# marcin119a/vae-los-angeles

Measured on AMD Instinct MI355X. Metric: training samples/sec, MultiModalVAE batch 65536, higher is better.
Workload: dtype bf16

## Files before the change

### include/mmvae_hip.h

```cpp
#ifndef MMVAE_HIP_H
#define MMVAE_HIP_H
#include <stdint.h>

#ifdef __cplusplus
extern "C" {
#endif

#define MMVAE_OK 0
#define MMVAE_ERR_ARG (-1)
#define MMVAE_ERR_DTYPE (-2)

enum { MMVAE_F32 = 0, MMVAE_BF16 = 1 };
enum { MMVAE_PREC_F32 = 0, MMVAE_PREC_BF16 = 1 };
enum { MMVAE_PRO_NONE = 0, MMVAE_PRO_BN_RELU_DROP = 1, MMVAE_PRO_BN_BWD_APPLY = 2 };
enum { MMVAE_EPI_STORE = 0, MMVAE_EPI_RELU_MASK = 1, MMVAE_EPI_BN_BWD = 2, MMVAE_EPI_LOSS_MSE = 3, MMVAE_EPI_LOSS_BCE_LOGIT = 4 };
enum { MMVAE_ACT_NONE = 0, MMVAE_ACT_RELU = 1, MMVAE_ACT_SIGMOID = 2 };

#define MMVAE_TILE 128

int mmvae_abi_version(void);
int mmvae_set_tuning(int32_t key, int32_t value);

typedef struct {
    const float* src; void* dst;
// ... 82 lines not shown

typedef struct {
    int32_t B, L, n_mod;
    const float* g_mu; const float* g_lv;
    const float* dz; const float* dz2; const float* dz3; int64_t lddz;
    const float* eps; const float* logvar;
    float* d_heads; int64_t ld_heads;
    float* d_table; const int64_t* site; int32_t S;
    void* d_heads_lp; int64_t ld_heads_lp;
    int32_t table_copies;
} mmvae_fuse_bwd_args;
#define MMVAE_TABLE_COPIES 8
int mmvae_fuse_reparam_bwd(const mmvae_fuse_bwd_args* args, void* stream);

typedef struct {
    int32_t B, A, D, S, L;
    const float* recon_a; const void* a; int64_t ld_ra, ld_a;
    const float* recon_b; const void* b; int64_t ld_rb, ld_b;
    const float* logits; int64_t ld_logits; const int64_t* site; const float* class_weights;
    const float* mu; const float* logvar;
    float beta, gamma;
    double* sums;
    void* g_a; int32_t g_a_dtype; int64_t ld_ga;
    void* g_b; int32_t g_b_dtype; int64_t ld_gb; int32_t grad_b_wrt_logit;
    float* g_c; int64_t ld_gc;
    float* g_mu; float* g_lv;
    const float* beta_gamma_dev;
    int32_t a_dtype, b_dtype;
} mmvae_loss_args;
int mmvae_vae_loss(const mmvae_loss_args* args, void* stream);
// ... 33 lines not shown
```

### vae-los-angeles_amd/csrc/common.h

```cpp
#pragma once
#include <hip/hip_runtime.h>
#include <stdint.h>
#include "mmvae_hip.h"

namespace mm {

typedef __bf16 bf16;
typedef __attribute__((ext_vector_type(8))) __bf16 bf16x8;
typedef __attribute__((ext_vector_type(4))) __bf16 bf16x4;
typedef __attribute__((ext_vector_type(4))) float f32x4;
typedef __attribute__((ext_vector_type(2))) float f32x2;
typedef __attribute__((ext_vector_type(4))) short s16x4;

constexpr int WAVE = 64;
constexpr int TILE = 128;
constexpr int NTHREADS = 256;
constexpr int ROW_BYTES = 128;

template <typename CT> struct Mma;

template <> struct Mma<bf16> {
    static constexpr int EPC = 8;
    static constexpr int KSTEP = 32;
    typedef bf16x8 frag;
// ... 123 lines not shown
#define STAMP_BUFFER(name)
#define STAMP_ENTRY()
#endif


struct Tuning {
    int nt_wide_min_m = 256 * 128;
    int nt2_on = 1;
    long split_bytes = 1L << 32;
    long block_bytes = 1L << 31;
    int tn_wide_on = 1;
    int bnbwd_stream = 1;
    int relu_stream = 1;
    int ntp_on = 1;
    int ntp_min_m = 16384;
};
inline Tuning g_tuning;

constexpr int NOT_TAKEN = 1 << 30;

template <auto Kernel, typename... Args>
inline int launch_lds(dim3 grid, dim3 block, int lds, hipStream_t st, const Args&... args) {
    static bool attr_done = false;
    if (!attr_done) {
        hipError_t e = hipFuncSetAttribute((const void*)Kernel, hipFuncAttributeMaxDynamicSharedMemorySize, lds);
        if (e != hipSuccess) return (int)e;
        attr_done = true;
    }
    hipLaunchKernelGGL(Kernel, grid, block, lds, st, args...);
    return (int)hipGetLastError();
// ... 49 lines not shown
```

### vae-los-angeles_amd/csrc/elementwise.hip

```cpp
#include <vector>
#include "common.h"
#include "mmvae_hip.h"

namespace mm {

__global__ __launch_bounds__(256) void prep_weights_kernel(const mmvae_prep_item* __restrict__ items) {
    const mmvae_prep_item it = items[blockIdx.y];
    __shared__ float tile[32][33];
    const int tx = threadIdx.x & 31, ty = threadIdx.x >> 5;
    const int tiles_c = (it.dst_cols + 31) / 32, tiles_r = (it.dst_rows + 31) / 32;
    auto put = [&](int r, int c, float v) {
        if (it.dst_dtype == MMVAE_BF16) ((bf16*)it.dst)[(long)r * it.dst_ld + c] = (bf16)v;
        else ((float*)it.dst)[(long)r * it.dst_ld + c] = v;
    };
    for (int t = blockIdx.x; t < tiles_r * tiles_c; t += gridDim.x) {
        const int tr = t / tiles_c, tc = t - tr * tiles_c;
        if (it.transpose) {
#pragma unroll
            for (int k = 0; k < 4; ++k) {
                const int sr = tc * 32 + ty + 8 * k, sc = tr * 32 + tx;
                tile[ty + 8 * k][tx] = (sr < it.src_rows && sc < it.src_cols) ? it.src[(long)sr * it.src_ld + sc] : 0.f;
            }
            __syncthreads();
#pragma unroll
// ... 189 lines not shown
    const float inv_n = 1.f / (float)a.n_mod;
    for (long i = (long)blockIdx.x * blockDim.x + threadIdx.x; i < total; i += (long)gridDim.x * blockDim.x) {
        const int b = (int)(i / a.ldz), l = (int)(i % a.ldz);
        ZT* zp = (ZT*)a.z + i;
        if (l >= a.L) { *zp = from_f32<ZT>(0.f); continue; }
        float mu = 0.f, lv = 0.f;
        if (a.heads_a) { mu += a.heads_a[(long)b * a.ld_heads + l]; lv += a.heads_a[(long)b * a.ld_heads + a.L + l]; }
        if (a.heads_b) { mu += a.heads_b[(long)b * a.ld_heads + l]; lv += a.heads_b[(long)b * a.ld_heads + a.L + l]; }
        if (a.table) {
            const long s = a.site[b];
            const bool ok = s >= 0 && s < a.S;
            const long sc = ok ? s : 0;
            const float bad = ok ? 0.f : __builtin_nanf("");
            mu += a.table[sc * 2 * a.L + l] + bad; lv += a.table[sc * 2 * a.L + a.L + l] + bad;
        }
        if (a.n_mod > 1) { mu *= inv_n; lv *= inv_n; }
        a.mu[(long)b * a.L + l] = mu; a.logvar[(long)b * a.L + l] = lv;
        *zp = from_f32<ZT>(mu + a.eps[(long)b * a.L + l] * expf(0.5f * lv));
    }
}

__global__ __launch_bounds__(256) void fuse_bwd_kernel(mmvae_fuse_bwd_args a, int rows_per_block, int use_lds) {
    extern __shared__ float sT[];
    const int L2 = 2 * a.L;
    if (use_lds) { for (int i = threadIdx.x; i < a.S * L2; i += blockDim.x) sT[i] = 0.f; __syncthreads(); }
    const int b0 = blockIdx.x * rows_per_block, b1 = min(a.B, b0 + rows_per_block);
    float* dtab = a.d_table ? a.d_table + (long)(blockIdx.x % (a.table_copies > 0 ? a.table_copies : 1)) * a.S * L2 : nullptr;
    const float inv_n = 1.f / (float)a.n_mod;
    constexpr int U = 4;
    const long iend = (long)b1 * a.L;
    for (long i0 = (long)b0 * a.L + threadIdx.x; i0 < iend; i0 += (long)U * blockDim.x) {
        float dz[U], gm[U], gl[U], ep[U], lv[U];
        int bb[U], ll[U];
// ... 772 lines not shown
```

### vae-los-angeles_amd/csrc/gemm_nt.hip

```cpp
#include "common.h"
#include "mmvae_hip.h"
#include "gemm_src.h"
#include "gemm_nt_epi.h"
#include "gemm_nt2.h"

namespace mm {

STAMP_BUFFER(nt)

__device__ __forceinline__ int swz(int row, int chunk) { return row * ROW_BYTES + ((chunk ^ (row & 7)) << 4); }

template <int WN> struct NtLds {
    static constexpr int BUF = (TILE + 64 * WN) * ROW_BYTES;
    static constexpr int STAGE = 2 * BUF;
    static constexpr int ECOL = STAGE + 4096 + 4 * 64 * WN * 4;
    static constexpr int TOTAL = ECOL + 8 * 64 * WN * 4;
};

template <typename CT, typename Src, typename Epi, int WN>
__global__ __launch_bounds__(128 * WN, 2)
void gemm_nt_kernel(Src src, const CT* __restrict__ W, long ldw, int M, int N, int K, int gx, int gy, Epi epi)
{
    constexpr int EPC = Mma<CT>::EPC;
    constexpr int BK = ROW_BYTES / (int)sizeof(CT);
// ... 245 lines not shown
                                    return launch_nt2<EpiLoss<MODE, VT, TT>, 2>(src.p, src.lda, a->w, a->ldw, a->M, a->N, a->K, e, st); }
#define MM_LOSS_VT(MODE, TT) { if (vt == 4) MM_LOSS_EPI(MODE, 4, TT) if (vt == 2) MM_LOSS_EPI(MODE, 2, TT) MM_LOSS_EPI(MODE, 1, TT) }
            if (h16) { if (mse) MM_LOSS_VT(0, bf16) MM_LOSS_VT(1, bf16) }
            if (mse) MM_LOSS_VT(0, float)
            MM_LOSS_VT(1, float)
#undef MM_LOSS_VT
#undef MM_LOSS_EPI
        }
        return MMVAE_ERR_ARG;
    }
    }
    return MMVAE_ERR_ARG;
}

BnFin bn_fin_of(const mmvae_gemm_nt_args* a) {
    BnFin f;
    if (!a->pro_finalize) return f;
    const mmvae_bn_finalize_args* b = (const mmvae_bn_finalize_args*)a->pro_finalize;
    f.sum = b->sum; f.sumsq = b->sumsq; f.gamma = b->gamma; f.beta = b->beta; f.eps = b->eps; f.momentum = b->momentum;
    f.running_mean = b->running_mean; f.running_var = b->running_var; f.nbt = (long long*)b->num_batches_tracked;
    f.mean = b->mean; f.rstd = b->rstd; f.scale = b->scale; f.shift = b->shift; f.M = b->M;
    return f;
}
static bool bn_fin_ok(const mmvae_gemm_nt_args* a) {
    if (!a->pro_finalize) return true;
    const mmvae_bn_finalize_args* b = (const mmvae_bn_finalize_args*)a->pro_finalize;
    return a->prologue == MMVAE_PRO_BN_RELU_DROP && b->N == a->K && b->M >= 2 && b->sum && b->sumsq && b->gamma && b->beta && b->mean && b->rstd && b->scale && b->shift;
}

template <typename CT>
static int dispatch_src(const mmvae_gemm_nt_args* a, hipStream_t st) {
    constexpr int EPC = Mma<CT>::EPC;
    if (a->prologue == MMVAE_PRO_BN_RELU_DROP) {
        if ((a->a_dtype == MMVAE_BF16) != (sizeof(CT) == 2)) return MMVAE_ERR_DTYPE;
        if (a->K > 512 || a->lda % EPC || ((uintptr_t)a->a & 15) || (!a->pro_finalize && (!a->pro_scale || !a->pro_shift))) return MMVAE_ERR_ARG;
        if (a->pro_mask && (a->ld_pro_mask % 4 || ((uintptr_t)a->pro_mask & 3))) return MMVAE_ERR_ARG;
        SrcBnReluDrop<CT> s{(const CT*)a->a, a->lda, a->M, a->K, a->pro_scale, a->pro_shift, a->pro_mask, a->ld_pro_mask, a->pro_inv_keep, bn_fin_of(a)};
// ... 15 lines not shown
extern "C" int mmvae_set_tuning(int32_t key, int32_t value) {
    mm::Tuning& t = mm::g_tuning;
    switch (key) {
    case 0: t.nt_wide_min_m = value; return 0;
    case 2: t.nt2_on = value; return 0;
    case 3:
        if (value != 0 && (value < 17 || value > 32)) return MMVAE_ERR_ARG;
        t.split_bytes = value ? 1L << value : mm::Tuning{}.split_bytes;
        t.block_bytes = t.split_bytes / 2;
        return 0;
    case 4: t.tn_wide_on = value; return 0;
    case 6: t.bnbwd_stream = value; return 0;
    case 7: t.relu_stream = value; return 0;
    case 8: t.ntp_on = value; return 0;
    case 9: t.ntp_min_m = value; return 0;
    }
    return MMVAE_ERR_ARG;
}

extern "C" int mmvae_gemm_nt(const mmvae_gemm_nt_args* a, void* stream) {
    if (!a || !a->a || !a->w || (!a->c && !(a->epilogue == MMVAE_EPI_BN_BWD && a->bn_phase == 0))) return MMVAE_ERR_ARG;
    if (a->M <= 0 || a->N <= 0 || a->K <= 0) return MMVAE_ERR_ARG;
    if (a->ldw % 64 || ((uintptr_t)a->w & 15)) return MMVAE_ERR_ARG;
    const long lim = 1L << 32;
    if (((long)a->N + 256) * a->ldw * 4 >= lim) return MMVAE_ERR_ARG;
    const long a_row = (long)a->lda * (a->a_dtype == MMVAE_BF16 ? 2 : 4);
    long row_bytes = a_row > (long)a->ld_pro_mask ? a_row : (long)a->ld_pro_mask;
    if (!mm::bn_fin_ok(a)) return MMVAE_ERR_ARG;
    if (mm::needs_row_blocks(a->M, row_bytes)) {
        if (a->pro_finalize || a->pro_out) return MMVAE_ERR_ARG;
// ... 23 lines not shown
```

### vae-los-angeles_amd/csrc/gemm_src.h

```cpp
#pragma once
#include "common.h"

namespace mm {

template <typename AT, int EPC> struct RawVec;
template <> struct RawVec<bf16, 8> {
    bf16x8 v;
    __device__ __forceinline__ float get(int i) const { return (float)v[i]; }
};
template <int EPC> struct RawVec<float, EPC> {
    float v[EPC];
    __device__ __forceinline__ float get(int i) const { return v[i]; }
};

template <int EPC, int VEC>
__device__ __forceinline__ void load_chunk_f32(RawVec<float, EPC>& r, const float* p, unsigned row_off, int k, int K) {
#pragma unroll
    for (int j = 0; j < EPC; j += VEC) VLoad<float, VEC>::ld(p + (row_off + (unsigned)min(k + j, K - VEC)), &r.v[j]);
}

template <typename CT, typename AT, int VEC>
struct SrcPlain {
    static constexpr int EPC = Mma<CT>::EPC;
    static constexpr bool NEEDS_AUX = false;
// ... 66 lines not shown
        if (var < 0.0) var = 0.0;
        const float rs = (float)(1.0 / sqrt(var + (double)eps));
        sc = gamma[i] * rs; sh = beta[i] - (float)mean_ * sc;
        if (first_wg) {
            mean[i] = (float)mean_; rstd[i] = rs; scale[i] = sc; shift[i] = sh;
            if (running_mean) {
                running_mean[i] = (1.f - momentum) * running_mean[i] + momentum * (float)mean_;
                const double unbiased = var * ((double)M / (double)(M - 1));
                running_var[i] = (1.f - momentum) * running_var[i] + momentum * (float)unbiased;
            }
            if (i == 0 && nbt) *nbt += 1;
        }
    }
};

template <typename CT>
struct SrcBnReluDrop {
    static constexpr int EPC = Mma<CT>::EPC;
    static constexpr bool NEEDS_AUX = true;
    static constexpr bool PAD_TAIL = false;
    const CT* y; long ldy; int M, K;
    const float* scale; const float* shift;
    const uint8_t* mask; long ldm; float inv_keep;
    BnFin fin = BnFin{};
    struct Raw { RawVec<CT, EPC> y; uint32_t m[EPC / 4]; };
    __device__ __forceinline__ void init(float* aux, int tid, int) const {
        if (fin.sum) {
            const bool first_wg = (blockIdx.x | blockIdx.y | blockIdx.z) == 0;
            for (int i = tid; i < K; i += NTHREADS) { float sc, sh; fin.column(i, first_wg, sc, sh); aux[i] = sc * inv_keep; aux[512 + i] = sh * inv_keep; }
            return;
// ... 84 lines not shown
```

### vae-los-angeles_amd/mmvae/_lib.py

```python
import ctypes as C
import os

_HERE = os.path.dirname(os.path.abspath(__file__))
LIB_PATH = os.environ.get("MMVAE_LIB_PATH") or os.path.join(_HERE, "libmmvae_hip.so")
ABI_VERSION = 20

F32, BF16 = 0, 1
PREC_F32, PREC_BF16 = 0, 1
PRO_NONE, PRO_BN_RELU_DROP, PRO_BN_BWD_APPLY = 0, 1, 2
TABLE_COPIES = 8
EPI_STORE, EPI_RELU_MASK, EPI_BN_BWD, EPI_LOSS_MSE, EPI_LOSS_BCE_LOGIT = 0, 1, 2, 3, 4
ACT_NONE, ACT_RELU, ACT_SIGMOID = 0, 1, 2
TILE = 128
TN_GROUP_MAX = 8
CTR_COPIES = 16384

i32, i64, f32, vp = C.c_int32, C.c_int64, C.c_float, C.c_void_p


class PrepItem(C.Structure):
    _fields_ = [("src", vp), ("dst", vp), ("src_rows", i32), ("src_cols", i32), ("src_ld", i64),
                ("dst_rows", i32), ("dst_cols", i32), ("dst_ld", i64), ("transpose", i32), ("dst_dtype", i32)]


# ... 38 lines not shown


class BnBwdFinalizeArgs(C.Structure):
    _fields_ = [("M", i32), ("N", i32), ("sum_d", vp), ("sum_dx", vp),
                ("gamma", vp), ("rstd", vp), ("dgamma", vp), ("dbeta", vp), ("coef", vp), ("eval_mode", i32)]


class FuseFwdArgs(C.Structure):
    _fields_ = [("B", i32), ("L", i32), ("n_mod", i32),
                ("heads_a", vp), ("heads_b", vp), ("ld_heads", i64),
                ("table", vp), ("site", vp), ("S", i32),
                ("eps", vp), ("mu", vp), ("logvar", vp),
                ("z", vp), ("z_dtype", i32), ("ldz", i64)]


class FuseBwdArgs(C.Structure):
    _fields_ = [("B", i32), ("L", i32), ("n_mod", i32),
                ("g_mu", vp), ("g_lv", vp), ("dz", vp), ("dz2", vp), ("dz3", vp), ("lddz", i64),
                ("eps", vp), ("logvar", vp),
                ("d_heads", vp), ("ld_heads", i64),
                ("d_table", vp), ("site", vp), ("S", i32), ("d_heads_lp", vp), ("ld_heads_lp", i64), ("table_copies", i32)]


class LossArgs(C.Structure):
    _fields_ = [("B", i32), ("A", i32), ("D", i32), ("S", i32), ("L", i32),
                ("recon_a", vp), ("a", vp), ("ld_ra", i64), ("ld_a", i64),
                ("recon_b", vp), ("b", vp), ("ld_rb", i64), ("ld_b", i64),
                ("logits", vp), ("ld_logits", i64), ("site", vp), ("class_weights", vp),
                ("mu", vp), ("logvar", vp),
                ("beta", f32), ("gamma", f32),
# ... 15 lines not shown
_SIGNATURES = {
    "mmvae_set_tuning": [i32, i32],
    "mmvae_prep_weights": [vp, i32, vp],
    "mmvae_gemm_nt": [C.POINTER(GemmNtArgs), vp],
    "mmvae_gemm_tn": [C.POINTER(GemmTnArgs), vp],
    "mmvae_gemm_tn_group": [vp, i32, vp],
    "mmvae_bn_finalize": [C.POINTER(BnFinalizeArgs), vp],
    "mmvae_bn_eval_coeffs": [i32, vp, vp, vp, vp, f32, vp, vp, vp, vp, vp],
    "mmvae_bn_bwd_finalize": [C.POINTER(BnBwdFinalizeArgs), vp],
    "mmvae_bn_bwd_apply": [i32, i32, i32, vp, i64, vp, i64, vp, vp, vp, vp],
    "mmvae_bn_bwd_finalize_apply": [i32, i32, i32, vp, i64, vp, i64, vp, vp, vp, vp, vp, vp, vp, i32, vp],
    "mmvae_embed_table_fwd": [i32, i32, i32, vp, vp, vp, vp, vp, vp, vp],
    "mmvae_embed_table_bwd": [i32, i32, i32, vp, vp, vp, vp, i32, vp, vp, vp, vp, vp, vp],
    "mmvae_fuse_reparam_fwd": [C.POINTER(FuseFwdArgs), vp],
    "mmvae_fuse_reparam_bwd": [C.POINTER(FuseBwdArgs), vp],
    "mmvae_vae_loss": [C.POINTER(LossArgs), vp],
    "mmvae_loss_finalize": [vp, f32, f32, vp, vp, vp],
    "mmvae_gather_rows": [vp, i32, vp, i32, i64, vp],
    "mmvae_rows_to_bf16": [vp, i32, i64, vp, i64, i32, i32, vp],
    "mmvae_sigmoid_bwd": [i32, i32, vp, i64, vp, i64, vp, i32, i64, vp],
    "mmvae_scale_if_needed": [vp, i32, i64, vp, vp],
    "mmvae_scale_many": [C.POINTER(ScaleItem), i32, vp, vp],
    "mmvae_noise": [vp, i64, f32, vp, i64, C.c_uint64, C.c_uint64, vp, i32, vp],
    "mmvae_counter_add": [vp, C.c_uint64, vp],
    "mmvae_adamw_step": [vp, i32, f32, f32, f32, f32, f32, f32, f32, i32, vp, i32, vp, vp],
}
EXPORTED = ["mmvae_abi_version"] + sorted(_SIGNATURES)

_lib = None

# ... 37 lines not shown
```

### vae-los-angeles_amd/mmvae/engine.py

```python
import os
from dataclasses import dataclass
from typing import NamedTuple, Optional

import torch

from . import ops
from . import _lib as L_
from .ops import (PREC_BF16, PREC_F32, ACT_NONE, ACT_RELU, ACT_SIGMOID, EPI_RELU_MASK, EPI_BN_BWD, DROP_P,
                  ceil_to, act_dtype, Prologue, BnBwdEpilogue, BnBwdFinalize, BnBwdApply)

_PRECISIONS = {"bf16": PREC_BF16, "fp32": PREC_F32, "f32": PREC_F32}
_default_precision = _PRECISIONS[os.environ.get("MMVAE_PRECISION", "bf16").lower()]
_TINY_DW_MAX = 16384


def set_default_precision(name):
    global _default_precision
    _default_precision = _PRECISIONS[name.lower()]


def default_precision():
    return _default_precision


# ... 184 lines not shown
        self.pl = [ops.PreparedLinear([l.weight], [l.bias], prec, device) for l in self.linears]
        self.pl_heads = ops.PreparedLinear([self.fc_mu.weight, self.fc_logvar.weight],
                                           [self.fc_mu.bias, self.fc_logvar.bias], prec, device)
        return self.pl + [self.pl_heads]

    def params(self):
        out = []
        for l, bn in zip(self.linears, self.bns):
            out += [l.weight, l.bias, bn.weight, bn.bias]
        out += [self.fc_mu.weight, self.fc_logvar.weight, self.fc_mu.bias, self.fc_logvar.bias]
        return out

    def widths(self):
        return [l.out_features for l in self.linears]

    def forward(self, prec, x, train, masks, stats_bufs=None, want_bwd=False):
        B, dev = x.shape[0], x.device
        adt = act_dtype(prec)
        layers = []
        h, pro = x, None
        fin = None

        def consume(N, K, out, bias, w, tag, stats=None, pro_out=None):
            nonlocal fin
            if fin is not None:
                try:
                    ops.gemm_nt(prec, h, w, N, K, out, bias=bias, prologue=pro, stats=stats, tag=tag, pro_out=pro_out, pro_finalize=fin)
                    fin = None
                    return pro_out
                except L_.MMVAEArgError:
                    pass
            if fin is not None:
                ops.bn_finalize_launch(fin)
                fin = None
            try:
                ops.gemm_nt(prec, h, w, N, K, out, bias=bias, prologue=pro, stats=stats, tag=tag, pro_out=pro_out)
                return pro_out
            except L_.MMVAEArgError:
                if pro_out is None:
                    raise
                ops.gemm_nt(prec, h, w, N, K, out, bias=bias, prologue=pro, stats=stats, tag=tag)
                return None

        for lin, bn, pl in zip(self.linears, self.bns, self.pl):
            N, K = pl.N, pl.K
            y = torch.empty(B, ceil_to(N, 8), dtype=adt, device=dev)
            st = BNState(N, dev)
            h_act = None
            if want_bwd and pro is not None and ops.can_keep_pro_out(prec, B, N, K, h, y) and pro.mask is not None \
                    and pro.mask.stride(0) % 8 == 0 and pro.mask.data_ptr() % 8 == 0:
                h_act = torch.empty(B, K, dtype=torch.bfloat16, device=dev)
            if train:
                stats = stats_bufs[len(layers)] if stats_bufs is not None else torch.zeros(2, N, dtype=torch.float64, device=dev)
                h_act = consume(N, K, y, pl.bias, pl.w, f"{self.name}.L{len(layers)}.fwd", stats=stats, pro_out=h_act)
                fin = ops.bn_finalize_args(B, N, stats, bn.weight, bn.bias, bn.running_mean, bn.running_var,
                                           bn.num_batches_tracked, st.mean, st.rstd, st.scale, st.shift, bn.eps,
                                           bn.momentum if bn.momentum is not None else 0.1)
                new_pro = Prologue(st.scale, st.shift, masks[len(layers)], 1.0 / (1.0 - DROP_P))
            else:
                ops.gemm_nt(prec, h, pl.w, N, K, y, bias=pl.bias, prologue=pro, tag=f"{self.name}.L{len(layers)}.fwd")
                ops.bn_eval_coeffs(bn.weight, bn.bias, bn.running_mean, bn.running_var, st.scale, st.shift, bn.eps, st.mean, st.rstd)
                new_pro = Prologue(st.scale, st.shift, None, 1.0)
            layers.append(LayerSave(h, pro, y, st, new_pro) if h_act is None else LayerSave(h_act, None, y, st, new_pro))
            h, pro = y, new_pro
        heads = torch.empty(B, 2 * self.latent, dtype=torch.float32, device=dev)
        consume(2 * self.latent, self.pl_heads.K, heads, self.pl_heads.bias, self.pl_heads.w, f"{self.name}.heads.fwd")
        return heads, layers

    def backward(self, prec, layers, d_heads, grads, tn=ops.gemm_tn, stats_bufs=None, train=True, d_heads_lp=None):
        B, dev = d_heads.shape[0], d_heads.device
        adt = act_dtype(prec)
        L2 = 2 * self.latent
        Kl = self.pl_heads.K
        gw = grads[self.fc_mu.weight]
        gb = grads[self.fc_mu.bias]
        tn(prec, d_heads, layers[-1].y, _span(gw, L2 * Kl).view(L2, Kl), _span(gb, L2), L2, Kl, q_prologue=layers[-1].y_prologue, tag=f"{self.name}.heads.dW")
        src, src_wt, src_n, src_k = (d_heads_lp if d_heads_lp is not None else d_heads), self.pl_heads.wt, Kl, L2
        for i in reversed(range(len(self.linears))):
            lin, bn, pl = self.linears[i], self.bns[i], self.pl[i]
            sv = layers[i]
            y = sv.y
            st = sv.bn
# ... 203 lines not shown

    def _forward(self, prec, xa, xb, site, train, want_bwd):
        ref = xa if xa is not None else (xb if xb is not None else site)
        dev, B = ref.device, ref.shape[0]
        self._prep.ensure(prec, dev, self.param_list(), self._prepare)
        state = StepState(prec, B, train)
        heads_a = heads_b = table = None
        Ld = self.latent
        widths_a = self.enc_a.widths() if (train and xa is not None) else []
        widths_b = self.enc_b.widths() if (train and xb is not None) else []
        n_a = len(widths_a)
        masks, eps = self.noise.draw(B, widths_a + widths_b, Ld, dev)
        zeros = self.zero_pack(dev, xa is not None, xb is not None, site is not None, fwd=True, bwd=want_bwd) if train else None
        if want_bwd:
            state.zeros = zeros
        if xa is not None:
            xa = _check_input(xa, "a", self.enc_a.in_dim, prec)
            heads_a, state.enc_a = self.enc_a.forward(prec, xa, train, masks[:n_a] if train else None,
                                                      zeros.fwd_stats[:n_a] if train else None, want_bwd=want_bwd)
        if xb is not None:
            xb = _check_input(xb.reshape(xb.shape[0], -1), "b", self.enc_b.in_dim, prec)
            heads_b, state.enc_b = self.enc_b.forward(prec, xb, train, masks[n_a:] if train else None,
                                                      zeros.fwd_stats[n_a:] if train else None, want_bwd=want_bwd)
        if site is not None:
            if site.dtype != torch.int64:
                site = site.long()
            site = site.contiguous()
            table = self.enc_c.table()
            state.site = site
        mu = torch.empty(B, Ld, dtype=torch.float32, device=dev)
        logvar = torch.empty(B, Ld, dtype=torch.float32, device=dev)
        z = torch.empty(B, ceil_to(Ld, 8), dtype=act_dtype(prec), device=dev)
        ops.fuse_reparam_fwd(B, Ld, heads_a, heads_b, table, site, eps, mu, logvar, z)
        state.eps, state.logvar = eps, logvar.detach()
        state.n_mod = (heads_a is not None) + (heads_b is not None) + (table is not None)
        outs, state.dec = [None] * len(self.decoders), [None] * len(self.decoders)
        order = sorted(range(len(self.decoders)), key=lambda i: -sum(l.weight.numel() for l in self.decoders[i].linears))
        stem = self.dec_stem
        firsts = [None] * len(self.decoders)
        if stem is not None:
            H0 = torch.empty(B, stem.N, dtype=act_dtype(prec), device=dev)
            ops.gemm_nt(prec, z, stem.w, stem.N, stem.K, H0, bias=stem.bias, act=ACT_RELU, tag="Decoders.L0.fwd")
            off = 0
            for i, d in enumerate(self.decoders):
                firsts[i] = H0[:, off:off + d.linears[0].out_features]
                off += d.linears[0].out_features
        fused = None
        want = self.fused_recon
        if want is not None and any(t is not None and self.decoders[i].can_fuse_loss(prec) for i, t in enumerate(want)):
            fused = state.fused = FusedRecon(*(zeros.loss_ws if want_bwd else ops.loss_workspace(dev)), {}, {})
        for i in order:
            dec = self.decoders[i]
            tgt = want[i] if (fused is not None and want[i] is not None and dec.can_fuse_loss(prec)) else None
            if tgt is not None:
                k = 1 if dec.final_sigmoid else 0
                g, acts = dec.forward(prec, z, fused_loss=(tgt, fused.sums[k:k + 1]), first=firsts[i])
                fused.g[i], fused.targets[i] = g, tgt
# ... 76 lines not shown
```

### vae-los-angeles_amd/mmvae/ops.py

```python
import ctypes as C
from collections import namedtuple

import torch

from . import _lib as L
from ._lib import (F32, BF16, PREC_F32, PREC_BF16, PRO_NONE, PRO_BN_RELU_DROP, PRO_BN_BWD_APPLY, EPI_STORE, EPI_RELU_MASK,
                   EPI_BN_BWD, EPI_LOSS_MSE, EPI_LOSS_BCE_LOGIT, ACT_NONE, ACT_RELU, ACT_SIGMOID, TILE)

DROP_P = 0.1
BN_EPS, BN_MOMENTUM = 1e-5, 0.1


class KernelProbe:

    def __init__(self, only=None):
        self.records = {}
        self.only = only

    def wants(self, tag):
        return tag is not None and (self.only is None or tag in self.only)

    def begin(self):
        ev = torch.cuda.Event(enable_timing=True)
        ev.record(torch.cuda.current_stream())
# ... 364 lines not shown
    L.check(L.load().mmvae_embed_table_bwd(S, E, w_mu.shape[0], emb.data_ptr(), w_mu.data_ptr(), w_lv.data_ptr(),
                                           d_table.data_ptr(), copies, d_emb.data_ptr(), d_w_mu.data_ptr(), d_b_mu.data_ptr(),
                                           d_w_lv.data_ptr(), d_b_lv.data_ptr(), _stream()), "mmvae_embed_table_bwd")


def fuse_reparam_fwd(B, Ld, heads_a, heads_b, table, site, eps, mu, logvar, z):
    n_mod = (heads_a is not None) + (heads_b is not None) + (table is not None)
    hd = heads_a if heads_a is not None else heads_b
    a = L.FuseFwdArgs(B, Ld, n_mod, _p(heads_a), _p(heads_b), _ld(hd) if hd is not None else 0,
                      _p(table), _p(site), table.shape[0] if table is not None else 0,
                      eps.data_ptr(), mu.data_ptr(), logvar.data_ptr(), z.data_ptr(), _dt(z), _ld(z))
    with stream_span("fuse_reparam_fwd", B * (8 * Ld * (n_mod - (table is not None)) + 8 * (table is not None) + 12 * Ld + z.element_size() * _ld(z))):
        L.check(L.load().mmvae_fuse_reparam_fwd(C.byref(a), _stream()), "mmvae_fuse_reparam_fwd")


def fuse_reparam_bwd(B, Ld, n_mod, g_mu, g_lv, dzs, eps, logvar, d_heads, d_table, site, d_heads_lp=None):
    dzs = list(dzs) + [None] * (3 - len(dzs))
    copies = d_table.shape[0] if (d_table is not None and d_table.dim() == 3) else 1
    a = L.FuseBwdArgs(B, Ld, n_mod, _p(g_mu), _p(g_lv), dzs[0].data_ptr(), _p(dzs[1]), _p(dzs[2]), _ld(dzs[0]), eps.data_ptr(), logvar.data_ptr(),
                      d_heads.data_ptr(), _ld(d_heads), _p(d_table), _p(site), d_table.shape[-2] if d_table is not None else 0,
                      _p(d_heads_lp), _ld(d_heads_lp) if d_heads_lp is not None else 0, copies)
    n_dz = sum(1 for d in dzs if d is not None)
    with stream_span("fuse_reparam_bwd", B * Ld * 4 * (n_dz + (g_mu is not None) + (g_lv is not None) + 2 + 2)):
        L.check(L.load().mmvae_fuse_reparam_bwd(C.byref(a), _stream()), "mmvae_fuse_reparam_bwd")


def loss_workspace(device):
    buf = torch.zeros(5 * 8 + 5 * 4 + 4, dtype=torch.uint8, device=device)
    return buf[:40].view(torch.float64), buf[40:60].view(torch.float32)

# ... 122 lines not shown
```

Measured before the change: 51.86 million.

## Fuse encoder heads, reparameterization and decoder stem into one latent kernel

Adds a single HIP kernel that applies the last encoder BN/ReLU/dropout prologue, computes both encoder head GEMMs, adds the site-embedding table, performs the reparameterization, writes mu/logvar/z, and runs the decoder stem GEMM with ReLU into H0. In the bf16 path this replaces separate head GEMMs, the fuse_reparam kernel and the stem GEMM, removing several launches and the round-trips of heads and z through global memory. If the kernel's argument checks fail, it falls back to the old sequence. The trade-offs are heavy LDS use and a persistent grid capped at 256 blocks, which may limit occupancy.

Measured after the change: 53.02 million (median of 6 runs). 2.3% higher.

```diff
diff --git a/include/mmvae_hip.h b/include/mmvae_hip.h
--- a/include/mmvae_hip.h
+++ b/include/mmvae_hip.h
@@ -120,6 +120,25 @@
 int mmvae_fuse_reparam_bwd(const mmvae_fuse_bwd_args* args, void* stream);
 
 typedef struct {
+    const void* y; int64_t ldy; int32_t K;
+    const float* scale; const float* shift;
+    const uint8_t* mask; int64_t ld_mask; float inv_keep;
+    const void* finalize;
+    const void* w; int64_t ldw; const float* bias;
+} mmvae_latent_enc;
+typedef struct {
+    int32_t prec, B, L, n_mod;
+    mmvae_latent_enc enc_a, enc_b;
+    const float* table; const int64_t* site; int32_t S;
+    const float* eps;
+    float* mu; float* logvar;
+    void* z; int64_t ldz;
+    const void* w_stem; int64_t ldw_stem; const float* bias_stem; int32_t N_stem;
+    void* h0; int64_t ldh0;
+} mmvae_latent_fwd_args;
+int mmvae_latent_fwd(const mmvae_latent_fwd_args* args, void* stream);
+
+typedef struct {
     int32_t B, A, D, S, L;
     const float* recon_a; const void* a; int64_t ld_ra, ld_a;
     const float* recon_b; const void* b; int64_t ld_rb, ld_b;
diff --git a/vae-los-angeles_amd/csrc/common.h b/vae-los-angeles_amd/csrc/common.h
--- a/vae-los-angeles_amd/csrc/common.h
+++ b/vae-los-angeles_amd/csrc/common.h
@@ -161,6 +161,7 @@
     int relu_stream = 1;
     int ntp_on = 1;
     int ntp_min_m = 16384;
+    int latent_on = 1;
 };
 inline Tuning g_tuning;
 
diff --git a/vae-los-angeles_amd/csrc/elementwise.hip b/vae-los-angeles_amd/csrc/elementwise.hip
--- a/vae-los-angeles_amd/csrc/elementwise.hip
+++ b/vae-los-angeles_amd/csrc/elementwise.hip
@@ -1,6 +1,7 @@
 #include <vector>
 #include "common.h"
 #include "mmvae_hip.h"
+#include "fuse_math.h"
 
 namespace mm {
 
@@ -227,9 +228,9 @@
             const float bad = ok ? 0.f : __builtin_nanf("");
             mu += a.table[sc * 2 * a.L + l] + bad; lv += a.table[sc * 2 * a.L + a.L + l] + bad;
         }
-        if (a.n_mod > 1) { mu *= inv_n; lv *= inv_n; }
+        const float zf = fuse_reparam_elem(mu, lv, a.n_mod, inv_n, a.eps[(long)b * a.L + l]);
         a.mu[(long)b * a.L + l] = mu; a.logvar[(long)b * a.L + l] = lv;
-        *zp = from_f32<ZT>(mu + a.eps[(long)b * a.L + l] * expf(0.5f * lv));
+        *zp = from_f32<ZT>(zf);
     }
 }
 
diff --git a/vae-los-angeles_amd/csrc/fuse_math.h b/vae-los-angeles_amd/csrc/fuse_math.h
--- /dev/null
+++ b/vae-los-angeles_amd/csrc/fuse_math.h
@@ -0,0 +1,11 @@
+#pragma once
+#include "common.h"
+
+namespace mm {
+
+__device__ __forceinline__ float fuse_reparam_elem(float& mu, float& lv, int n_mod, float inv_n, float eps) {
+    if (n_mod > 1) { mu *= inv_n; lv *= inv_n; }
+    return mu + eps * expf(0.5f * lv);
+}
+
+}
diff --git a/vae-los-angeles_amd/csrc/gemm_nt.hip b/vae-los-angeles_amd/csrc/gemm_nt.hip
--- a/vae-los-angeles_amd/csrc/gemm_nt.hip
+++ b/vae-los-angeles_amd/csrc/gemm_nt.hip
@@ -283,13 +283,7 @@
 }
 
 BnFin bn_fin_of(const mmvae_gemm_nt_args* a) {
-    BnFin f;
-    if (!a->pro_finalize) return f;
-    const mmvae_bn_finalize_args* b = (const mmvae_bn_finalize_args*)a->pro_finalize;
-    f.sum = b->sum; f.sumsq = b->sumsq; f.gamma = b->gamma; f.beta = b->beta; f.eps = b->eps; f.momentum = b->momentum;
-    f.running_mean = b->running_mean; f.running_var = b->running_var; f.nbt = (long long*)b->num_batches_tracked;
-    f.mean = b->mean; f.rstd = b->rstd; f.scale = b->scale; f.shift = b->shift; f.M = b->M;
-    return f;
+    return bn_fin_from((const mmvae_bn_finalize_args*)a->pro_finalize);
 }
 static bool bn_fin_ok(const mmvae_gemm_nt_args* a) {
     if (!a->pro_finalize) return true;
@@ -335,6 +329,7 @@
     case 7: t.relu_stream = value; return 0;
     case 8: t.ntp_on = value; return 0;
     case 9: t.ntp_min_m = value; return 0;
+    case 10: t.latent_on = value; return 0;
     }
     return MMVAE_ERR_ARG;
 }
diff --git a/vae-los-angeles_amd/csrc/gemm_src.h b/vae-los-angeles_amd/csrc/gemm_src.h
--- a/vae-los-angeles_amd/csrc/gemm_src.h
+++ b/vae-los-angeles_amd/csrc/gemm_src.h
@@ -104,6 +104,15 @@
     }
 };
 
+inline BnFin bn_fin_from(const mmvae_bn_finalize_args* b) {
+    BnFin f;
+    if (!b) return f;
+    f.sum = b->sum; f.sumsq = b->sumsq; f.gamma = b->gamma; f.beta = b->beta; f.eps = b->eps; f.momentum = b->momentum;
+    f.running_mean = b->running_mean; f.running_var = b->running_var; f.nbt = (long long*)b->num_batches_tracked;
+    f.mean = b->mean; f.rstd = b->rstd; f.scale = b->scale; f.shift = b->shift; f.M = b->M;
+    return f;
+}
+
 template <typename CT>
 struct SrcBnReluDrop {
     static constexpr int EPC = Mma<CT>::EPC;
diff --git a/vae-los-angeles_amd/csrc/latent.hip b/vae-los-angeles_amd/csrc/latent.hip
--- /dev/null
+++ b/vae-los-angeles_amd/csrc/latent.hip
@@ -0,0 +1,250 @@
+#include "common.h"
+#include "mmvae_hip.h"
+#include "gemm_src.h"
+#include "fuse_math.h"
+
+namespace mm {
+
+constexpr int LAT_WAVES = 8, LAT_THREADS = 64 * LAT_WAVES;
+constexpr int LAT_NK = 8;
+constexpr int LAT_HN = 48;
+constexpr int LAT_FU = LAT_HN / 2 * 16 / 64;
+constexpr int LAT_NS = 448;
+constexpr int LAT_MAXTAB = 1024;
+constexpr int LAT_WROW = LAT_NK * 64 + 16;
+constexpr int LAT_SROW = 64 + 16;
+constexpr int LAT_SUMLD = 52;
+constexpr int LAT_OFF_WS = 2 * LAT_HN * LAT_WROW;
+constexpr int LAT_OFF_AUX = LAT_OFF_WS + LAT_NS * LAT_SROW;
+constexpr int LAT_OFF_BIAS = LAT_OFF_AUX + 2 * 4096;
+constexpr int LAT_OFF_TAB = LAT_OFF_BIAS + (2 * LAT_HN + LAT_NS) * 4;
+constexpr int LAT_OFF_SCR = LAT_OFF_TAB + LAT_MAXTAB * 4;
+constexpr int LAT_SCR_Z = 16 * LAT_SUMLD * 4;
+constexpr int LAT_SCR = LAT_SCR_Z + 16 * LAT_SROW;
+constexpr int LAT_LDS = LAT_OFF_SCR + LAT_WAVES * LAT_SCR;
+
+struct LatEnc { SrcBnReluDrop<bf16> src; const bf16* w; long ldw; const float* bias; int nk; };
+struct LatArgs {
+    LatEnc e[2];
+    int B, L, n_mod, S;
+    const float* table; const long long* site; const float* eps; float* mu; float* logvar;
+    bf16* z; long ldz;
+    const bf16* ws; long ldws; const float* bs; int ns;
+    bf16* h0; long ldh0;
+    int nslabs;
+};
+
+__device__ __forceinline__ void lat_wave_sync() { asm volatile("s_waitcnt lgkmcnt(0)" ::: "memory"); __builtin_amdgcn_wave_barrier(); }
+
+__global__ __launch_bounds__(LAT_THREADS) void latent_fwd_kernel(const LatArgs a) {
+    typedef SrcBnReluDrop<bf16>::Raw Raw;
+    extern __shared__ __attribute__((aligned(16))) unsigned char smem[];
+    const int tid = threadIdx.x, lane = tid & 63, wid = tid >> 6;
+    const int li = lane & 15, lg = lane >> 4;
+    float* const aux = (float*)(smem + LAT_OFF_AUX);
+    float* const sbias = (float*)(smem + LAT_OFF_BIAS);
+    float* const stab = (float*)(smem + LAT_OFF_TAB);
+    unsigned char* const scr = smem + LAT_OFF_SCR + wid * LAT_SCR;
+    float* const ssum = (float*)scr;
+    unsigned char* const sz = scr + LAT_SCR_Z;
+    const int L = a.L, L2 = 2 * a.L;
+    const bool any_enc = a.e[0].nk + a.e[1].nk > 0;
+
+    int fr[LAT_FU], fl[LAT_FU];
+#pragma unroll
+    for (int i = 0; i < LAT_FU; ++i) { const int x = lane + 64 * i; fr[i] = x / L; fl[i] = x - fr[i] * L; }
+    const int zcpr = (int)(a.ldz >> 3), zr = lane / zcpr, zc = lane - zr * zcpr;
+    const float inv_n = 1.f / (float)a.n_mod;
+    const int total = a.B * L;
+
+    Raw raw[2][LAT_NK];
+    float eps_r[LAT_FU];
+    long long site_r[LAT_FU] = {};
+    auto fetch = [&](int slab) __attribute__((always_inline)) {
+        const int row = slab * 16 + li;
+#pragma unroll
+        for (int e = 0; e < 2; ++e)
+#pragma unroll
+            for (int j = 0; j < LAT_NK; ++j)
+                if (j < a.e[e].nk) a.e[e].src.fetch(raw[e][j], row, 32 * j + 8 * lg);
+#pragma unroll
+        for (int i = 0; i < LAT_FU; ++i) {
+            const int idx = min(slab * 16 * L + lane + 64 * i, total - 1);
+            eps_r[i] = a.eps[idx];
+        }
+        if (a.table) {
+#pragma unroll
+            for (int i = 0; i < LAT_FU; ++i) site_r[i] = a.site[min(slab * 16 + fr[i], a.B - 1)];
+        }
+    };
+
+    const int nw = gridDim.x * LAT_WAVES;
+    int slab = blockIdx.x * LAT_WAVES + wid;
+    if (slab < a.nslabs) fetch(slab);
+
+#pragma unroll
+    for (int e = 0; e < 2; ++e) {
+        if (a.e[e].nk == 0) continue;
+        static_assert(NTHREADS <= LAT_THREADS && 32 * LAT_NK <= 512, "SrcBnReluDrop's table: 512 columns, filled by NTHREADS threads");
+        if (tid < NTHREADS) a.e[e].src.init(aux + e * 1024, tid, 0);
+        const int cpr = a.e[e].nk * 4;
+        for (int c = tid; c < LAT_HN * cpr; c += LAT_THREADS) {
+            const int r = c / cpr, ch = c - r * cpr;
+            *(uint4*)(smem + (e * LAT_HN + r) * LAT_WROW + ch * 16) = *(const uint4*)(a.e[e].w + (long)r * a.e[e].ldw + ch * 8);
+        }
+        if (tid < LAT_HN) sbias[e * LAT_HN + tid] = (a.e[e].bias && tid < L2) ? a.e[e].bias[tid] : 0.f;
+    }
+    for (int c = tid; c < a.ns * 4; c += LAT_THREADS) {
+        const int x = c >> 2, ch = c & 3, q = (x >> 4) & 3, i = x & 15;
+        const int wr = (x & ~63) + 32 * (q >> 1) + 8 * (i >> 2) + 4 * (q & 1) + (i & 3);
+        *(uint4*)(smem + LAT_OFF_WS + x * LAT_SROW + ch * 16) = *(const uint4*)(a.ws + (long)wr * a.ldws + ch * 8);
+    }
+    for (int c = tid; c < a.ns; c += LAT_THREADS) sbias[2 * LAT_HN + c] = a.bs ? a.bs[c] : 0.f;
+    if (a.table) for (int i = tid; i < a.S * L2; i += LAT_THREADS) stab[i] = a.table[i];
+    for (int i = lane; i < 16 * LAT_SROW / 16; i += 64) ((uint4*)sz)[i] = uint4{0u, 0u, 0u, 0u};
+    __syncthreads();
+
+    for (; slab < a.nslabs; slab += nw) {
+        f32x4 hs[3];
+#pragma unroll
+        for (int e = 0; e < 2; ++e) {
+            if (a.e[e].nk == 0) continue;
+            f32x4 acc[3];
+#pragma unroll
+            for (int n = 0; n < 3; ++n) acc[n] = f32x4{0.f, 0.f, 0.f, 0.f};
+#pragma unroll
+            for (int j = 0; j < LAT_NK; ++j) {
+                if (j >= a.e[e].nk) break;
+                Chunk<bf16> o;
+                a.e[e].src.finish_fast(raw[e][j], 32 * j + 8 * lg, o, aux + e * 1024);
+#pragma unroll
+                for (int n = 0; n < 3; ++n) {
+                    const bf16x8 wf = *(const bf16x8*)(smem + (e * LAT_HN + 16 * n + li) * LAT_WROW + (4 * j + lg) * 16);
+                    Mma<bf16>::mma(acc[n], wf, o.v);
+                }
+            }
+#pragma unroll
+            for (int n = 0; n < 3; ++n) {
+                const f32x4 h = acc[n] + *(const f32x4*)(sbias + e * LAT_HN + 16 * n + 4 * lg);
+                hs[n] = (e == 1 && a.e[0].nk) ? hs[n] + h : h;
+            }
+        }
+        if (any_enc) {
+#pragma unroll
+            for (int n = 0; n < 3; ++n) *(f32x4*)(ssum + li * LAT_SUMLD + 16 * n + 4 * lg) = hs[n];
+        }
+        float ep[LAT_FU];
+        long long st[LAT_FU];
+#pragma unroll
+        for (int i = 0; i < LAT_FU; ++i) { ep[i] = eps_r[i]; st[i] = site_r[i]; }
+        if (slab + nw < a.nslabs) fetch(slab + nw);
+        lat_wave_sync();
+
+#pragma unroll
+        for (int i = 0; i < LAT_FU; ++i) {
+            if (lane + 64 * i >= 16 * L) break;
+            const int r = fr[i], l = fl[i];
+            float mu = 0.f, lv = 0.f;
+            if (any_enc) { mu += ssum[r * LAT_SUMLD + l]; lv += ssum[r * LAT_SUMLD + L + l]; }
+            if (a.table) {
+                const long long s = st[i];
+                const bool ok = s >= 0 && s < a.S;
+                const int sc = ok ? (int)s : 0;
+                const float bad = ok ? 0.f : __builtin_nanf("");
+                mu += stab[sc * L2 + l] + bad; lv += stab[sc * L2 + L + l] + bad;
+            }
+            const float zf = fuse_reparam_elem(mu, lv, a.n_mod, inv_n, ep[i]);
+            const int idx = slab * 16 * L + lane + 64 * i;
+            if (idx < total) { a.mu[idx] = mu; a.logvar[idx] = lv; }
+            ((bf16*)sz)[r * (LAT_SROW / 2) + l] = (bf16)zf;
+        }
+        lat_wave_sync();
+        if (lane < 16 * zcpr && slab * 16 + zr < a.B)
+            *(uint4*)(a.z + (long)(slab * 16 + zr) * a.ldz + zc * 8) = *(const uint4*)(sz + zr * LAT_SROW + zc * 16);
+
+        const bf16x8 zf8 = *(const bf16x8*)(sz + li * LAT_SROW + lg * 16);
+        const bool lowl = li < 8;
+        const int rbase = slab * 16 + (li & 7);
+        bf16* const crow = a.h0 + (long)rbase * a.ldh0 + 32 * (li >> 3) + 8 * lg;
+        const bool ok0 = rbase < a.B, ok1 = rbase + 8 < a.B;
+        for (int p = 0; p < (a.ns >> 6); ++p) {
+            f32x4 acc[4];
+#pragma unroll
+            for (int q = 0; q < 4; ++q) {
+                const bf16x8 wf = *(const bf16x8*)(smem + LAT_OFF_WS + (64 * p + 16 * q + li) * LAT_SROW + lg * 16);
+                acc[q] = f32x4{0.f, 0.f, 0.f, 0.f};
+                Mma<bf16>::mma(acc[q], wf, zf8);
+            }
+            uint32_t pk[2][4];
+#pragma unroll
+            for (int h = 0; h < 2; ++h) {
+                const float* bp = sbias + 2 * LAT_HN + 64 * p + 32 * h + 8 * lg;
+                const f32x4 b0 = *(const f32x4*)bp, b1 = *(const f32x4*)(bp + 4);
+                const f32x4 x0 = acc[2 * h] + b0, x1 = acc[2 * h + 1] + b1;
+#pragma unroll
+                for (int qd = 0; qd < 4; ++qd) {
+                    const f32x4 x = qd < 2 ? x0 : x1;
+                    typedef __attribute__((ext_vector_type(2))) __bf16 bf16x2;
+                    const bf16x2 t = {(bf16)fmaxf(x[2 * (qd & 1)], 0.f), (bf16)fmaxf(x[2 * (qd & 1) + 1], 0.f)};
+                    pk[h][qd] = __builtin_bit_cast(uint32_t, t);
+                }
+            }
+            uint32_t st0[4], st1[4];
+#pragma unroll
+            for (int qd = 0; qd < 4; ++qd) {
+                const uint32_t send = lowl ? pk[1][qd] : pk[0][qd];
+                const uint32_t got = (uint32_t)__builtin_amdgcn_mov_dpp((int)send, 0x128, 0xf, 0xf, true);
+                st0[qd] = lowl ? pk[0][qd] : got;
+                st1[qd] = lowl ? got : pk[1][qd];
+            }
+            if (ok0) *(uint4*)(crow + 64 * p) = uint4{st0[0], st0[1], st0[2], st0[3]};
+            if (ok1) *(uint4*)(crow + 8 * a.ldh0 + 64 * p) = uint4{st1[0], st1[1], st1[2], st1[3]};
+        }
+        lat_wave_sync();
+    }
+}
+
+static int lat_enc(const mmvae_latent_enc& e, int B, LatEnc& o) {
+    o = LatEnc{};
+    if (!e.y) return 0;
+    const mmvae_bn_finalize_args* f = (const mmvae_bn_finalize_args*)e.finalize;
+    if (e.K < 32 || e.K % 32 || e.K > 32 * LAT_NK || e.ldy % 8 || e.ldy < e.K || ((uintptr_t)e.y & 15)) return MMVAE_ERR_ARG;
+    if (!e.w || e.ldw % 64 || e.ldw < e.K || ((uintptr_t)e.w & 15)) return MMVAE_ERR_ARG;
+    if (!f && (!e.scale || !e.shift)) return MMVAE_ERR_ARG;
+    if (f && (f->N != e.K || f->M != B || B < 2 || !f->sum || !f->sumsq || !f->gamma || !f->beta || !f->mean || !f->rstd || !f->scale || !f->shift))
+        return MMVAE_ERR_ARG;
+    if (e.mask && (e.ld_mask % 8 || e.ld_mask < e.K || ((uintptr_t)e.mask & 7))) return MMVAE_ERR_ARG;
+    const long lim = 1L << 32;
+    if ((long)B * e.ldy * 2 >= lim || (e.mask && (long)B * e.ld_mask >= lim)) return MMVAE_ERR_ARG;
+    o.src = SrcBnReluDrop<bf16>{(const bf16*)e.y, e.ldy, B, e.K, e.scale, e.shift, e.mask, e.ld_mask, e.inv_keep, bn_fin_from(f)};
+    o.w = (const bf16*)e.w; o.ldw = e.ldw; o.bias = e.bias; o.nk = e.K / 32;
+    return 0;
+}
+
+}
+
+extern "C" int mmvae_latent_fwd(const mmvae_latent_fwd_args* a, void* stream) {
+    using namespace mm;
+    if (!a || !g_tuning.latent_on) return MMVAE_ERR_ARG;
+    if (a->prec != MMVAE_PREC_BF16) return MMVAE_ERR_DTYPE;
+    if (a->B <= 0 || a->L <= 0 || 2 * a->L > LAT_HN || (long)a->B * a->L >= (1L << 31)) return MMVAE_ERR_ARG;
+    if (!a->eps || !a->mu || !a->logvar || !a->z || !a->w_stem || !a->h0) return MMVAE_ERR_ARG;
+    const int present = (a->enc_a.y != nullptr) + (a->enc_b.y != nullptr) + (a->table != nullptr);
+    if (present == 0 || present != a->n_mod) return MMVAE_ERR_ARG;
+    if (a->table && (!a->site || a->S <= 0 || (long)a->S * 2 * a->L > LAT_MAXTAB)) return MMVAE_ERR_ARG;
+    if (a->ldz % 8 || a->ldz < a->L || a->ldz > 32 || ((uintptr_t)a->z & 15)) return MMVAE_ERR_ARG;
+    if (a->N_stem < 64 || a->N_stem % 64 || a->N_stem > LAT_NS || a->ldw_stem % 64 || a->ldw_stem < 32 || ((uintptr_t)a->w_stem & 15)) return MMVAE_ERR_ARG;
+    if (a->ldh0 % 64 || a->ldh0 < a->N_stem || ((uintptr_t)a->h0 & 127) || (long)a->B * a->ldh0 * 2 >= (1L << 32)) return MMVAE_ERR_ARG;
+    LatArgs k{};
+    { const int rc = lat_enc(a->enc_a, a->B, k.e[0]); if (rc) return rc; }
+    { const int rc = lat_enc(a->enc_b, a->B, k.e[1]); if (rc) return rc; }
+    k.B = a->B; k.L = a->L; k.n_mod = a->n_mod; k.S = a->S;
+    k.table = a->table; k.site = (const long long*)a->site; k.eps = a->eps; k.mu = a->mu; k.logvar = a->logvar;
+    k.z = (bf16*)a->z; k.ldz = a->ldz;
+    k.ws = (const bf16*)a->w_stem; k.ldws = a->ldw_stem; k.bs = a->bias_stem; k.ns = a->N_stem;
+    k.h0 = (bf16*)a->h0; k.ldh0 = a->ldh0;
+    k.nslabs = (a->B + 15) / 16;
+    int grid = (k.nslabs + LAT_WAVES - 1) / LAT_WAVES;
+    if (grid > 256) grid = 256;
+    return launch_lds<latent_fwd_kernel>(dim3(grid), dim3(LAT_THREADS), LAT_LDS, (hipStream_t)stream, k);
+}
diff --git a/vae-los-angeles_amd/mmvae/_lib.py b/vae-los-angeles_amd/mmvae/_lib.py
--- a/vae-los-angeles_amd/mmvae/_lib.py
+++ b/vae-los-angeles_amd/mmvae/_lib.py
@@ -76,6 +76,22 @@
                 ("z", vp), ("z_dtype", i32), ("ldz", i64)]
 
 
+class LatentEnc(C.Structure):
+    _fields_ = [("y", vp), ("ldy", i64), ("K", i32), ("scale", vp), ("shift", vp),
+                ("mask", vp), ("ld_mask", i64), ("inv_keep", f32), ("finalize", vp),
+                ("w", vp), ("ldw", i64), ("bias", vp)]
+
+
+class LatentFwdArgs(C.Structure):
+    _fields_ = [("prec", i32), ("B", i32), ("L", i32), ("n_mod", i32),
+                ("enc_a", LatentEnc), ("enc_b", LatentEnc),
+                ("table", vp), ("site", vp), ("S", i32),
+                ("eps", vp), ("mu", vp), ("logvar", vp),
+                ("z", vp), ("ldz", i64),
+                ("w_stem", vp), ("ldw_stem", i64), ("bias_stem", vp), ("N_stem", i32),
+                ("h0", vp), ("ldh0", i64)]
+
+
 class FuseBwdArgs(C.Structure):
     _fields_ = [("B", i32), ("L", i32), ("n_mod", i32),
                 ("g_mu", vp), ("g_lv", vp), ("dz", vp), ("dz2", vp), ("dz3", vp), ("lddz", i64),
@@ -121,6 +137,7 @@
     "mmvae_embed_table_bwd": [i32, i32, i32, vp, vp, vp, vp, i32, vp, vp, vp, vp, vp, vp],
     "mmvae_fuse_reparam_fwd": [C.POINTER(FuseFwdArgs), vp],
     "mmvae_fuse_reparam_bwd": [C.POINTER(FuseBwdArgs), vp],
+    "mmvae_latent_fwd": [C.POINTER(LatentFwdArgs), vp],
     "mmvae_vae_loss": [C.POINTER(LossArgs), vp],
     "mmvae_loss_finalize": [vp, f32, f32, vp, vp, vp],
     "mmvae_gather_rows": [vp, i32, vp, i32, i64, vp],
diff --git a/vae-los-angeles_amd/mmvae/engine.py b/vae-los-angeles_amd/mmvae/engine.py
--- a/vae-los-angeles_amd/mmvae/engine.py
+++ b/vae-los-angeles_amd/mmvae/engine.py
@@ -222,34 +222,29 @@
     def widths(self):
         return [l.out_features for l in self.linears]
 
-    def forward(self, prec, x, train, masks, stats_bufs=None, want_bwd=False):
+    def _consume(self, prec, h, pro, fin, N, K, out, bias, w, tag, stats=None, pro_out=None):
+        if fin is not None:
+            try:
+                ops.gemm_nt(prec, h, w, N, K, out, bias=bias, prologue=pro, stats=stats, tag=tag, pro_out=pro_out, pro_finalize=fin)
+                return pro_out
+            except L_.MMVAEArgError:
+                pass
+            ops.bn_finalize_launch(fin)
+        try:
+            ops.gemm_nt(prec, h, w, N, K, out, bias=bias, prologue=pro, stats=stats, tag=tag, pro_out=pro_out)
+            return pro_out
+        except L_.MMVAEArgError:
+            if pro_out is None:
+                raise
+            ops.gemm_nt(prec, h, w, N, K, out, bias=bias, prologue=pro, stats=stats, tag=tag)
+            return None
+
+    def forward(self, prec, x, train, masks, stats_bufs=None, want_bwd=False, heads=True):
         B, dev = x.shape[0], x.device
         adt = act_dtype(prec)
         layers = []
         h, pro = x, None
         fin = None
-
-        def consume(N, K, out, bias, w, tag, stats=None, pro_out=None):
-            nonlocal fin
-            if fin is not None:
-                try:
-                    ops.gemm_nt(prec, h, w, N, K, out, bias=bias, prologue=pro, stats=stats, tag=tag, pro_out=pro_out, pro_finalize=fin)
-                    fin = None
-                    return pro_out
-                except L_.MMVAEArgError:
-                    pass
-            if fin is not None:
-                ops.bn_finalize_launch(fin)
-                fin = None
-            try:
-                ops.gemm_nt(prec, h, w, N, K, out, bias=bias, prologue=pro, stats=stats, tag=tag, pro_out=pro_out)
-                return pro_out
-            except L_.MMVAEArgError:
-                if pro_out is None:
-                    raise
-                ops.gemm_nt(prec, h, w, N, K, out, bias=bias, prologue=pro, stats=stats, tag=tag)
-                return None
-
         for lin, bn, pl in zip(self.linears, self.bns, self.pl):
             N, K = pl.N, pl.K
             y = torch.empty(B, ceil_to(N, 8), dtype=adt, device=dev)
@@ -260,7 +255,7 @@
                 h_act = torch.empty(B, K, dtype=torch.bfloat16, device=dev)
             if train:
                 stats = stats_bufs[len(layers)] if stats_bufs is not None else torch.zeros(2, N, dtype=torch.float64, device=dev)
-                h_act = consume(N, K, y, pl.bias, pl.w, f"{self.name}.L{len(layers)}.fwd", stats=stats, pro_out=h_act)
+                h_act = self._consume(prec, h, pro, fin, N, K, y, pl.bias, pl.w, f"{self.name}.L{len(layers)}.fwd", stats=stats, pro_out=h_act)
                 fin = ops.bn_finalize_args(B, N, stats, bn.weight, bn.bias, bn.running_mean, bn.running_var,
                                            bn.num_batches_tracked, st.mean, st.rstd, st.scale, st.shift, bn.eps,
                                            bn.momentum if bn.momentum is not None else 0.1)
@@ -271,9 +266,14 @@
                 new_pro = Prologue(st.scale, st.shift, None, 1.0)
             layers.append(LayerSave(h, pro, y, st, new_pro) if h_act is None else LayerSave(h_act, None, y, st, new_pro))
             h, pro = y, new_pro
-        heads = torch.empty(B, 2 * self.latent, dtype=torch.float32, device=dev)
-        consume(2 * self.latent, self.pl_heads.K, heads, self.pl_heads.bias, self.pl_heads.w, f"{self.name}.heads.fwd")
-        return heads, layers
+        owed = ops.LatentEncoder(h, pro, fin, self.pl_heads)
+        return (self.run_heads(prec, owed) if heads else owed), layers
+
+    def run_heads(self, prec, owed):
+        heads = torch.empty(owed.y.shape[0], 2 * self.latent, dtype=torch.float32, device=owed.y.device)
+        self._consume(prec, owed.y, owed.prologue, owed.fin, 2 * self.latent, self.pl_heads.K, heads, self.pl_heads.bias, self.pl_heads.w,
+                      f"{self.name}.heads.fwd")
+        return heads
 
     def backward(self, prec, layers, d_heads, grads, tn=ops.gemm_tn, stats_bufs=None, train=True, d_heads_lp=None):
         B, dev = d_heads.shape[0], d_heads.device
@@ -507,14 +507,16 @@
         zeros = self.zero_pack(dev, xa is not None, xb is not None, site is not None, fwd=True, bwd=want_bwd) if train else None
         if want_bwd:
             state.zeros = zeros
+        stem = self.dec_stem
+        fuse_latent = stem is not None and prec == PREC_BF16
         if xa is not None:
             xa = _check_input(xa, "a", self.enc_a.in_dim, prec)
             heads_a, state.enc_a = self.enc_a.forward(prec, xa, train, masks[:n_a] if train else None,
-                                                      zeros.fwd_stats[:n_a] if train else None, want_bwd=want_bwd)
+                                                      zeros.fwd_stats[:n_a] if train else None, want_bwd=want_bwd, heads=not fuse_latent)
         if xb is not None:
             xb = _check_input(xb.reshape(xb.shape[0], -1), "b", self.enc_b.in_dim, prec)
             heads_b, state.enc_b = self.enc_b.forward(prec, xb, train, masks[n_a:] if train else None,
-                                                      zeros.fwd_stats[n_a:] if train else None, want_bwd=want_bwd)
+                                                      zeros.fwd_stats[n_a:] if train else None, want_bwd=want_bwd, heads=not fuse_latent)
         if site is not None:
             if site.dtype != torch.int64:
                 site = site.long()
@@ -524,16 +526,24 @@
         mu = torch.empty(B, Ld, dtype=torch.float32, device=dev)
         logvar = torch.empty(B, Ld, dtype=torch.float32, device=dev)
         z = torch.empty(B, ceil_to(Ld, 8), dtype=act_dtype(prec), device=dev)
-        ops.fuse_reparam_fwd(B, Ld, heads_a, heads_b, table, site, eps, mu, logvar, z)
+        H0 = torch.empty(B, stem.N, dtype=act_dtype(prec), device=dev) if stem is not None else None
+        if fuse_latent:
+            try:
+                ops.latent_fwd(prec, B, Ld, heads_a, heads_b, table, site, eps, mu, logvar, z, stem, H0)
+            except L_.MMVAEArgError:
+                fuse_latent = False
+                heads_a = self.enc_a.run_heads(prec, heads_a) if heads_a is not None else None
+                heads_b = self.enc_b.run_heads(prec, heads_b) if heads_b is not None else None
+        if not fuse_latent:
+            ops.fuse_reparam_fwd(B, Ld, heads_a, heads_b, table, site, eps, mu, logvar, z)
         state.eps, state.logvar = eps, logvar.detach()
         state.n_mod = (heads_a is not None) + (heads_b is not None) + (table is not None)
         outs, state.dec = [None] * len(self.decoders), [None] * len(self.decoders)
         order = sorted(range(len(self.decoders)), key=lambda i: -sum(l.weight.numel() for l in self.decoders[i].linears))
-        stem = self.dec_stem
         firsts = [None] * len(self.decoders)
         if stem is not None:
-            H0 = torch.empty(B, stem.N, dtype=act_dtype(prec), device=dev)
-            ops.gemm_nt(prec, z, stem.w, stem.N, stem.K, H0, bias=stem.bias, act=ACT_RELU, tag="Decoders.L0.fwd")
+            if not fuse_latent:
+                ops.gemm_nt(prec, z, stem.w, stem.N, stem.K, H0, bias=stem.bias, act=ACT_RELU, tag="Decoders.L0.fwd")
             off = 0
             for i, d in enumerate(self.decoders):
                 firsts[i] = H0[:, off:off + d.linears[0].out_features]
diff --git a/vae-los-angeles_amd/mmvae/ops.py b/vae-los-angeles_amd/mmvae/ops.py
--- a/vae-los-angeles_amd/mmvae/ops.py
+++ b/vae-los-angeles_amd/mmvae/ops.py
@@ -402,6 +402,45 @@
         L.check(L.load().mmvae_fuse_reparam_fwd(C.byref(a), _stream()), "mmvae_fuse_reparam_fwd")
 
 
+LatentEncoder = namedtuple("LatentEncoder", "y prologue fin heads")
+
+
+def _latent_enc(e, enc):
+    sc, sh, mask, inv_keep = enc.prologue
+    e.y, e.ldy, e.K = _mat(enc.y, "y").data_ptr(), _ld(enc.y), enc.heads.K
+    e.scale, e.shift, e.mask, e.ld_mask, e.inv_keep = sc.data_ptr(), sh.data_ptr(), _p(mask), (_ld(mask) if mask is not None else 0), inv_keep
+    if enc.fin is not None:
+        e.finalize = C.addressof(enc.fin)
+    e.w, e.ldw, e.bias = enc.heads.w.data_ptr(), enc.heads.w.stride(0), _p(enc.heads.bias)
+
+
+def latent_fwd_args(prec, B, Ld, enc_a, enc_b, table, site, eps, mu, logvar, z, stem, h0):
+    a = L.LatentFwdArgs()
+    a.prec, a.B, a.L = prec, B, Ld
+    a.n_mod = (enc_a is not None) + (enc_b is not None) + (table is not None)
+    nbytes = 12 * Ld + z.element_size() * _ld(z) + h0.element_size() * stem.N + 8 * (table is not None)
+    for e, enc in ((a.enc_a, enc_a), (a.enc_b, enc_b)):
+        if enc is not None:
+            _latent_enc(e, enc)
+            nbytes += enc.heads.K * (enc.y.element_size() + (enc.prologue[2] is not None))
+    if table is not None:
+        a.table, a.site, a.S = table.data_ptr(), _p(site), table.shape[0]
+    a.eps, a.mu, a.logvar = eps.data_ptr(), mu.data_ptr(), logvar.data_ptr()
+    a.z, a.ldz = z.data_ptr(), _ld(z)
+    a.w_stem, a.ldw_stem, a.bias_stem, a.N_stem = stem.w.data_ptr(), stem.w.stride(0), _p(stem.bias), stem.N
+    a.h0, a.ldh0 = h0.data_ptr(), _ld(h0)
+    return a, B * nbytes
+
+
+def latent_fwd(prec, B, Ld, enc_a, enc_b, table, site, eps, mu, logvar, z, stem, h0):
+    for t in (eps, mu, logvar):
+        if tuple(t.shape) != (B, Ld) or not t.is_contiguous():
+            raise ValueError(f"latent_fwd: eps / mu / logvar must be contiguous ({B}, {Ld}), got {tuple(t.shape)} / {t.stride()}")
+    a, nbytes = latent_fwd_args(prec, B, Ld, enc_a, enc_b, table, site, eps, mu, logvar, z, stem, h0)
+    with stream_span("latent.fwd", nbytes):
+        L.check(L.load().mmvae_latent_fwd(C.byref(a), _stream()), "mmvae_latent_fwd")
+
+
 def fuse_reparam_bwd(B, Ld, n_mod, g_mu, g_lv, dzs, eps, logvar, d_heads, d_table, site, d_heads_lp=None):
     dzs = list(dzs) + [None] * (3 - len(dzs))
     copies = d_table.shape[0] if (d_table is not None and d_table.dim() == 3) else 1
```
